# CILAB-MA/gpudrive_lab

Measured on AMD Instinct MI355X. Metric: agent-steps/sec at 1024 worlds x 64 agents; achieved HBM GB/s on obs kernel, higher is better.
Workload: dtype f32

## Files before the change

gpudrive_lab_amd/csrc/engine.cpp:

```cpp
#include <hip/hip_runtime.h>

#include <algorithm>
#include <cmath>
#include <cstdlib>
#include <cstdio>
#include <cstring>
#include <map>
#include <memory>
#include <stdexcept>
#include <atomic>
#include <exception>
#include <string>
#include <thread>
#include <vector>

#include "dev_mem.hpp"
#include "engine.hpp"
#include "gd_math.hpp"
#include "scene.hpp"
#ifdef GD_CLOCKS
namespace gd { void set_clocks_read(unsigned long long *out); void step_clocks_read(unsigned long long *out); }
#endif
#ifndef GD_GRID_MIN_CELL
#define GD_GRID_MIN_CELL 16.f
// ... 127 lines not shown
    std::vector<int32_t> deleted;
    std::vector<WorldHost> world_host;
    int cu_count = 256;
    Growable<float2, 320, 640> road_xy;
    Growable<Float8, 320, 640> road_aux, road_rec;
    Growable<gd::RoadBox, 0, 64> boxes;
    Growable<int32_t, 0, 64> cell_off, cell_items;
    Growable<float4, 0, 64> cell_hdr;
    Growable<int32_t, 0, 64> rcell_off;
    Growable<uint16_t, 64, 128> rcell_items, rcell_pos;
    Growable<float2, 64, 128> rcell_xy;
    Growable<float4, 0, 64> road_blk;
    int32_t *d_road_off = nullptr, *d_box_off = nullptr, *d_blk_off = nullptr;
    gd::GridHdr *d_grid = nullptr, *d_rgrid = nullptr;
    float4 *d_road_bbox = nullptr;
    float *d_road_rbmax = nullptr;
    static constexpr int kRing = 8;
    PinnedFlags h_flags[kRing];
    Event flag_ev[kRing];
    int ring_pos = 0;
    static constexpr size_t kEvRing = 32;
    Stream side;
    Event ev_fork, ev_join;
    size_t lin_cap = 0;
    int32_t *d_row_of_slot = nullptr, *d_slot_of_row = nullptr, *d_row_count = nullptr;
    int32_t *d_lin_list = nullptr, *d_lin_list_dyn = nullptr;
    bool full_pass_next = false;
    int64_t lin_static_agents = 0;
    int64_t host_skipped = 0;
    bool rk_possible = false;
    bool rk_alloc = false;

    bool ensure_rank_buffers() {
        if (rk_alloc) return true;
        const size_t WA = static_cast<size_t>(W) * A;
        std::vector<gd::DevMem> mine;
        gd::DevSim n = d;
        try {
            alloc_into(mine, n.rk_E, WA * GD_RANK_CAP + 64);
            alloc_into(mine, n.rk_spc, WA * GD_RANK_SPL);
            if (std::getenv("GPUDRIVE_RANK_ALLOC_FAIL") != nullptr)
                throw HipError("GPUDRIVE_RANK_ALLOC_FAIL: simulated allocation failure of the rank replay's buffers");
            alloc_into(mine, n.rk_kt, WA * GD_RANK_KT);
            alloc_into(mine, n.rk_heap, WA * GD_RANK_HEAP_DW);
            alloc_into(mine, n.rk_cpe, WA * GD_RANK_NCP);
            alloc_into(mine, n.rk_n, WA);
            alloc_into(mine, n.rk_fallback, WA / 32);
            alloc_into(mine, n.rk_streak, WA / 32);
            alloc_into(mine, n.cp_road, 2 * WA * GD_RANK_NCP);
            alloc_into(mine, n.cp_T, 2 * WA * GD_RANK_NCP);
            alloc_into(mine, n.cp_hdr, 2 * WA);
            alloc_into(mine, n.rk_cp, WA * GD_RANK_NCP);
            alloc_into(mine, n.rk_tl, WA);
            alloc_into(mine, n.rk_hist, 544);
            alloc_into(mine, n.rk_ticket, WA);
            alloc_into(mine, n.rk_order, WA);
            alloc_into(mine, n.rk_list, 8 * WA);
            n.rk_nlong = static_cast<int>(std::max<size_t>(WA / 4, 64));
            alloc_into(mine, n.rk_longlist, n.rk_nlong);
            alloc_into(mine, n.rk_longslot, WA);
            alloc_into(mine, n.rk_E_long, static_cast<size_t>(n.rk_nlong) * GD_RANK_CAP_LONG + 64);
            alloc_into(mine, n.rk_kt_long, static_cast<size_t>(n.rk_nlong) * GD_RANK_KT_LONG);
            internal.reserve(internal.size() + mine.size());
        } catch (const HipError &) {
            (void)hipGetLastError();
            rk_possible = false;
            d.rk_on = 0;
            return false;
        }
        for (gd::DevMem &m : mine) internal.push_back(std::move(m));
        d = n;
        rk_alloc = true;
        return true;
    }
    bool timing = false;
    std::vector<EventPair> ev_pool[gd::KERNEL_TIMED];
    size_t ev_head[gd::KERNEL_TIMED] = {};
    size_t ev_used[gd::KERNEL_TIMED] = {};
    double ev_ms[gd::KERNEL_TIMED] = {};
    int64_t ev_launches[gd::KERNEL_TIMED] = {};

    ~gd_sim() {
        (void)hipDeviceSynchronize();
        if (step_graph) (void)hipGraphExecDestroy(step_graph);
    }

    template <typename T>
    static void alloc_into(std::vector<gd::DevMem> &into, T *&field, size_t count) {
        const size_t bytes = std::max<size_t>(count * sizeof(T), 16);
        into.emplace_back(bytes);
        HIP_CHECK(hipMemset(into.back().get(), 0, bytes));
        field = static_cast<T *>(into.back().get());
    }
    template <typename T>
    T *alloc_internal(size_t count) {
        T *p = nullptr;
        alloc_into(internal, p, count);
        return p;
    }

    void collect_timing(int k, size_t keep = 0) {
        while (ev_used[k] > keep) {
            const EventPair &e = ev_pool[k][ev_head[k]];
            float ms = 0.f;
            if (hipEventSynchronize(e.stop.get()) == hipSuccess && hipEventElapsedTime(&ms, e.start.get(), e.stop.get()) == hipSuccess) {
                ev_ms[k] += ms;
                ev_launches[k]++;
// ... 523 lines not shown
            for (int c = 0; c < nc; c++) off[c + 1] += off[c];
            std::vector<int32_t> fill(off.begin(), off.end() - 1);
            for (size_t r = 0; r < n; r++) items[fill[cell_of[r]]++] = static_cast<uint16_t>(r);
        }
        world.rgrid = g;
        world.rcell_off = std::move(off);
        world.rcell_items = std::move(items);
    }

    void upload_road_grids() {
        size_t ncell = 0, nitem = 0;
        std::vector<gd::GridHdr> hdr(W);
        for (int w = 0; w < W; w++) {
            world_host[w].rgrid.cell_base = static_cast<int>(ncell);
            world_host[w].rgrid.item_base = static_cast<int>(nitem);
            hdr[w] = world_host[w].rgrid;
            ncell += world_host[w].rcell_off.size();
            nitem += world_host[w].rcell_items.size();
        }
        rcell_off.fit(ncell, d.rcell_off);
        rcell_items.fit(nitem, d.rcell_items);
        rcell_xy.fit(nitem, d.rcell_xy);
        rcell_pos.fit(nitem, d.rcell_pos);
        std::vector<int32_t> co(ncell);
        std::vector<uint16_t> ci(nitem);
        std::vector<float> cxy(nitem * 2);
        std::vector<uint16_t> cpos(nitem);
        for (int w = 0; w < W; w++) {
            const WorldHost &x = world_host[w];
            std::copy(x.rcell_off.begin(), x.rcell_off.end(), co.begin() + hdr[w].cell_base);
            std::copy(x.rcell_items.begin(), x.rcell_items.end(), ci.begin() + hdr[w].item_base);
            for (size_t k = 0; k < x.rcell_items.size(); k++) {
                const size_t r = x.rcell_items[k], o = (static_cast<size_t>(hdr[w].item_base) + k) * 2;
                cxy[o] = x.xy[2 * r];
                cxy[o + 1] = x.xy[2 * r + 1];
                cpos[static_cast<size_t>(hdr[w].item_base) + r] = static_cast<uint16_t>(k);
            }
        }
        rcell_off.upload(co.data(), ncell);
        rcell_items.upload(ci.data(), nitem);
        rcell_xy.upload(cxy.data(), nitem);
        rcell_pos.upload(cpos.data(), nitem);
        HIP_CHECK(hipMemcpy(d_rgrid, hdr.data(), sizeof(gd::GridHdr) * W, hipMemcpyHostToDevice));
        std::vector<float> prev(static_cast<size_t>(W) * A * 4, 0.f);
        for (size_t i = 0; i < static_cast<size_t>(W) * A; i++) prev[i * 4 + 2] = INFINITY;
        HIP_CHECK(hipMemcpy(d.knn_prev, prev.data(), prev.size() * sizeof(float), hipMemcpyHostToDevice));
    }

    void reset_rank_state() {
        HIP_CHECK(hipMemset(d.cp_hdr, 0, sizeof(float4) * 2 * static_cast<size_t>(W) * A));
        HIP_CHECK(hipMemset(d.rk_fallback, 0, sizeof(int32_t) * (static_cast<size_t>(W) * A / 32)));
        HIP_CHECK(hipMemset(d.rk_streak, 0, sizeof(int32_t) * (static_cast<size_t>(W) * A / 32)));
        HIP_CHECK(hipMemset(d.rk_hist, 0, sizeof(int32_t) * GD_RANK_AUDIT));
    }

    void do_reset(const std::vector<int32_t> &flags) {
        upload_flags(d.reset_flags, flags);
        reset_flagged(false);
    }

    void reset_flagged(bool gated) {
        d.gate_any = gated ? 1 : 0;
        if (!gated) full_pass_next = false;
        try {
            launch(gd::KERNEL_RESET, false);
            run_rest(false);
        } catch (...) {
            d.gate_any = 0;
            throw;
        }
        d.gate_any = 0;
    }
};

namespace {

template <typename F>
int guarded(F &&f) {
    try {
        f();
        return GD_OK;
    } catch (const HipError &e) {
        return fail(GD_ERR_DEVICE, e.what());
    } catch (const std::invalid_argument &e) {
        const std::string m = e.what();
        return fail(m.find("cannot open") != std::string::npos ? GD_ERR_IO : GD_ERR_INVALID, m);
    } catch (const std::exception &e) {
        return fail(GD_ERR_PARSE, e.what());
    }
}

}

extern "C" {

const char *gd_version(void) { return "gpudrive_amd 0.1 (gfx950)"; }
const char *gd_last_error(void) { return g_last_error.c_str(); }

void gd_default_params(gd_params *p) {
    std::memset(p, 0, sizeof(*p));
    p->collisionBehaviour = GD_COLLISION_AGENT_STOP;
    p->maxNumControlledAgents = 10000;
    p->IgnoreNonVehicles = 0;
    p->roadObservationAlgorithm = GD_ROADS_K_NEAREST;
    p->initOnlyValidAgentsAtFirstStep = 1;
    p->isStaticAgentControlled = 0;
// ... 105 lines not shown
        d.resp = s->alloc_internal<int32_t>(WA);
        d.sel_idx = s->alloc_internal<uint16_t>(static_cast<size_t>(WA) * GD_MAP_OBS_K);
        d.sel_hdr = s->alloc_internal<float4>(static_cast<size_t>(WA) * 2);
        d.sel_slot = s->alloc_internal<uint8_t>(static_cast<size_t>(WA) * GD_MAP_OBS_K);
        d.reset_flags = s->alloc_internal<int32_t>(W);
        d.rebuilt_flags = s->alloc_internal<int32_t>(W);
        d.any_reset = s->alloc_internal<int32_t>(1);
        d.gate_any = 0;
        d.road_off = s->d_road_off = s->alloc_internal<int32_t>(W + 1);
        d.live_list = s->alloc_internal<int32_t>(WA);
        d.live_count = 0;
        d.set_groups = s->alloc_internal<int32_t>(WA);
        d.set_group_count = 0;
        d.wave_order = s->alloc_internal<int32_t>(static_cast<size_t>(W) * (A / GD_MAP_OBS_AW));
        d.wave_cost = s->alloc_internal<uint32_t>(static_cast<size_t>(W) * (A / GD_MAP_OBS_AW));
        d.box_off = s->d_box_off = s->alloc_internal<int32_t>(W + 1);
        d.grid = s->d_grid = s->alloc_internal<gd::GridHdr>(W);
        d.rgrid = s->d_rgrid = s->alloc_internal<gd::GridHdr>(W);
        d.knn_prev = s->alloc_internal<float4>(WA);
        d.road_bbox = s->d_road_bbox = s->alloc_internal<float4>(W);
        d.road_rbmax = s->d_road_rbmax = s->alloc_internal<float>(W);
        d.bev_dirty = s->alloc_internal<int32_t>(WA);
        d.bev_list = s->alloc_internal<int32_t>(WA);
        d.bev_count = s->alloc_internal<int32_t>(2);
        d.bev_all_dirty = 0;
        HIP_CHECK(hipMemset(d.bev_dirty, 1, sizeof(int32_t) * WA));
        d.lidar_dirty = s->alloc_internal<int32_t>(WA);
        d.lidar_head = s->alloc_internal<float>(WA);
        HIP_CHECK(hipMemset(d.lidar_dirty, 1, sizeof(int32_t) * WA));
        HIP_CHECK(hipMemset(d.lidar_head, 0xff, sizeof(float) * WA));
        d.lin_apw = 2;
        if (const char *e = std::getenv("GPUDRIVE_LIN_AGENTS_PER_WAVE")) d.lin_apw = std::min(A / 4, std::max(1, std::atoi(e)));
        s->lin_cap = (static_cast<size_t>(W) + 64) * static_cast<size_t>(A) + 8 * 4 * static_cast<size_t>(d.lin_apw) + 64;
        s->d_lin_list = s->alloc_internal<int32_t>(s->lin_cap);
        s->d_lin_list_dyn = s->alloc_internal<int32_t>(s->lin_cap);
        d.lin_list = s->d_lin_list; d.lin_list_dyn = s->d_lin_list_dyn;
        d.lin_blocks = 0; d.lin_blocks_dyn = 0; d.lin_dyn_off = 0;
        d.lin_on = std::getenv("GPUDRIVE_LINEAR_LEGACY") == nullptr ? 1 : 0;
        d.pose_stamp = s->alloc_internal<uint4>(WA);
        d.pose_skip = std::getenv("GPUDRIVE_NO_POSE_SKIP") == nullptr ? 1 : 0;
        d.stat_skipped = s->alloc_internal<unsigned long long>(GD_SKIP_SLOTS);
        s->d_row_of_slot = s->alloc_internal<int32_t>(WA);
        s->d_slot_of_row = s->alloc_internal<int32_t>(WA);
        s->d_row_count = s->alloc_internal<int32_t>(1);
        d.bad_actions = s->alloc_internal<unsigned long long>(1);
        d.blk_off = s->d_blk_off = s->alloc_internal<int32_t>(W + 1);
        d.warm_k = 0;
        d.warm_all = 0;
        d.warm_flags = s->alloc_internal<int32_t>(W);
        d.warm_count = s->alloc_internal<unsigned long long>(1);
        d.rk_on = 0;
        d.rk_dbg = 0;
        d.rk_min_roads = 1536;
        s->rk_possible = GD_MAP_OBS_AW == 32 && cfg->knn_order != GD_KNN_SET_ORDER &&
                         params->roadObservationAlgorithm == GD_ROADS_K_NEAREST && std::getenv("GPUDRIVE_NO_RANK_REPLAY") == nullptr;
#ifdef GD_DIAG
        if (const char *e = std::getenv("GPUDRIVE_RANK_DBG")) d.rk_dbg = std::atoi(e);
#endif
        for (int i = 0; i < gd_sim::kRing; i++) {
            void *pinned = nullptr;
            HIP_CHECK(hipHostMalloc(&pinned, sizeof(int32_t) * W, hipHostMallocDefault));
            s->h_flags[i].reset(static_cast<int32_t *>(pinned));
            s->flag_ev[i] = make_event(hipEventDisableTiming);
        }
        std::vector<int> all(W);
        for (int w = 0; w < W; w++) all[w] = w;
        s->rebuild_worlds(all);
        s->do_reset(std::vector<int32_t>(W, 1));
        HIP_CHECK(hipStreamSynchronize(s->stream));
    });
    if (rc != GD_OK) return rc;
    *out = s.release();
    return GD_OK;
}

void gd_destroy(gd_sim *sim) { delete sim; }

int gd_step(gd_sim *s) {
    if (!s) return fail(GD_ERR_INVALID, "gd_step: null sim");
    return guarded([&]() { s->step(); });
}

int gd_reset(gd_sim *s, const int32_t *idx, int32_t n) {
    if (!s || (n > 0 && !idx)) return fail(GD_ERR_INVALID, "gd_reset: bad argument");
    std::vector<int32_t> flags(s->W, 0);
    for (int i = 0; i < n; i++) {
        if (idx[i] < 0 || idx[i] >= s->W) return fail(GD_ERR_INVALID, "gd_reset: world index out of range");
        flags[idx[i]] = 1;
    }
    return guarded([&]() { s->do_reset(flags); });
}

int gd_set_maps(gd_sim *s, const char *const *scenes, int32_t n) {
    if (!s || !scenes) return fail(GD_ERR_INVALID, "gd_set_maps: null argument");
    if (n != s->W) return fail(GD_ERR_INVALID, "gd_set_maps: len(maps) must equal the number of worlds");
    const std::vector<std::string> old_scenes = s->scenes;
    const std::vector<int32_t> old_deleted = s->deleted;
    const int rc = guarded([&]() {
        for (int w = 0; w < n; w++) {
            if (!scenes[w]) throw std::invalid_argument("gd_set_maps: null scene path");
            s->scenes[w] = scenes[w];
        }
        std::fill(s->deleted.begin(), s->deleted.end(), -1);
        std::vector<int> all(s->W);
        for (int w = 0; w < s->W; w++) all[w] = w;
        s->rebuild_worlds(all);
// ... 1070 lines not shown
    if (!s) return fail(GD_ERR_INVALID, "gd_set_stream: null sim");
    return guarded([&]() {
        HIP_CHECK(hipStreamSynchronize(s->stream));
        s->drop_graph();
        HIP_CHECK(hipStreamSynchronize(s->side.get()));
        s->stream = static_cast<hipStream_t>(stream);
        s->d.split_partner = (s->stream != nullptr && std::getenv("GPUDRIVE_SPLIT_PARTNER") != nullptr) ? 1 : 0;
    });
}

int gd_attach_bev(gd_sim *s, float *bev) {
    if (!s || !bev) return fail(GD_ERR_INVALID, "gd_attach_bev: null argument");
    return guarded([&]() {
        if (s->d.bev && s->d.bev != bev) throw std::runtime_error("gd_attach_bev: a BEV tensor is already attached");
        HIP_CHECK(hipStreamSynchronize(s->stream));
        s->drop_graph();
        s->exported[GD_T_BEV] = bev;
        s->d.bev = bev;
        HIP_CHECK(hipMemsetAsync(s->d.bev_dirty, 1, sizeof(int32_t) * static_cast<size_t>(s->W) * s->A, s->stream));
        if (!s->params.disableClassicalObs) s->launch(gd::KERNEL_BEV, false);
    });
}

int gd_stat(gd_sim *s, int32_t which, int64_t *out) {
#ifdef GD_CLOCKS
    if (s && out && which >= 22 && which <= 29) {
        static unsigned long long clk[8];
        if (which == 22) gd::set_clocks_read(clk);
        *out = (int64_t)clk[which - 22];
        return GD_OK;
    }
#endif
#ifdef GD_CLOCKS
    if (s && out && which >= 32 && which <= 43) {
        static unsigned long long clk[12];
        if (which == 32) gd::step_clocks_read(clk);
        *out = (int64_t)clk[which - 32];
        return GD_OK;
    }
#endif
#ifdef GD_CLOCKS
    if (s && out && which >= 1000 && which < 1256) {
        *out = 0;
        if (s->rk_alloc) {
            int32_t v = 0;
            (void)hipStreamSynchronize(s->stream);
            if (hipMemcpy(&v, s->d.rk_hist + 256 + (which - 1000), sizeof(v), hipMemcpyDeviceToHost) != hipSuccess)
                return fail(GD_ERR_DEVICE, "gd_stat: reading the replay clocks failed");
            *out = v;
        }
        return GD_OK;
    }
#endif
#if defined(GD_DIAG) || defined(GD_CLOCKS)
    constexpr int32_t kLastStat = 20;
#else
    constexpr int32_t kLastStat = 7;
#endif
    if (s && out && which == 30) {
        std::vector<unsigned long long> v(GD_SKIP_SLOTS, 0);
        (void)hipStreamSynchronize(s->stream);
        if (hipMemcpy(v.data(), s->d.stat_skipped, sizeof(unsigned long long) * v.size(), hipMemcpyDeviceToHost) != hipSuccess ||
            hipMemset(s->d.stat_skipped, 0, sizeof(unsigned long long) * v.size()) != hipSuccess)
            return fail(GD_ERR_DEVICE, "gd_stat: reading the skip counters failed");
        unsigned long long sum = 0;
        for (unsigned long long x : v) sum += x;
        *out = static_cast<int64_t>(sum) + s->host_skipped;
        s->host_skipped = 0;
        return GD_OK;
    }
    if (s && out && which == 31) {
        int32_t c = 0;
        (void)hipStreamSynchronize(s->stream);
        if (hipMemcpy(&c, s->d.bev_count, sizeof(c), hipMemcpyDeviceToHost) != hipSuccess)
            return fail(GD_ERR_DEVICE, "gd_stat: reading the raster count failed");
        *out = c;
        return GD_OK;
    }
    if (s && out && which == 44) {
        std::vector<int32_t> f(static_cast<size_t>(s->W) * s->A), n(static_cast<size_t>(s->W) * 2);
        (void)hipStreamSynchronize(s->stream);
        if (hipMemcpy(f.data(), s->d.lidar_dirty, sizeof(int32_t) * f.size(), hipMemcpyDeviceToHost) != hipSuccess ||
            hipMemcpy(n.data(), s->d.shape, sizeof(int32_t) * n.size(), hipMemcpyDeviceToHost) != hipSuccess)
            return fail(GD_ERR_DEVICE, "gd_stat: reading the LiDAR flags failed");
        int64_t c = 0;
        for (int w = 0; w < s->W; w++)
            for (int a = 0; a < n[static_cast<size_t>(w) * 2] && a < s->A; a++) c += f[static_cast<size_t>(w) * s->A + a] != 0;
        *out = c;
        return GD_OK;
    }
    if (s && out && which == 45) {
        unsigned long long v = 0;
        (void)hipStreamSynchronize(s->stream);
        if (hipMemcpy(&v, s->d.bad_actions, sizeof(v), hipMemcpyDeviceToHost) != hipSuccess)
            return fail(GD_ERR_DEVICE, "gd_stat: reading the action counter failed");
        *out = static_cast<int64_t>(v);
        return GD_OK;
    }
    if (s && out && which == 46) {
        unsigned long long v = 0;
        (void)hipStreamSynchronize(s->stream);
        if (hipMemcpy(&v, s->d.warm_count, sizeof(v), hipMemcpyDeviceToHost) != hipSuccess)
            return fail(GD_ERR_DEVICE, "gd_stat: reading the warm-up counter failed");
        *out = static_cast<int64_t>(v);
        return GD_OK;
    }
// ... 180 lines not shown
```

gpudrive_lab_amd/csrc/engine.hpp:

```cpp
#pragma once
#include <hip/hip_runtime.h>

#include <cstdint>

#include "../../include/gpudrive_amd.h"

#ifndef GD_MAP_OBS_AW
#define GD_MAP_OBS_AW 32
#endif

#define GD_RANK_CAP 1280
#define GD_RANK_NCP 40
#define GD_RANK_HEAP_DW 104
#define GD_RANK_CAP_LONG 2560
#define GD_RANK_KT_LONG 164
#define GD_RH_LONG 537
#define GD_RANK_NCH 320
#define GD_RANK_SPL 256
#define GD_RANK_KT 84
#define GD_RANK_AUDIT 536
#define GD_LIN_BLK 16
#define GD_SKIP_SLOTS 4096

#ifdef GD_DIAG
#define GD_DIAG_IS(field, value) ((field) == (value))
#else
#define GD_DIAG_IS(field, value) false
#endif

namespace gd {

enum { KERNEL_STATE = 0, KERNEL_MAP_OBS = 1, KERNEL_LIDAR = 2, KERNEL_BEV = 3, KERNEL_PARTNER = 4, KERNEL_RESET = 5, KERNEL_PADDING = 6, KERNEL_TIMED = 5 };

struct GridHdr {
    float ox, oy, inv_cell;
    int nx, ny;
    int cell_base;
    int item_base;
    int pad;
};

struct DevSim {
    int W, A;
    int knn_order;
    int set_fused_rows;
    int32_t *live_list;
    int live_count;
    int32_t *set_groups;
    int set_group_count;
    int set_apw;
    float lidar_half_angle;
    float radius_key_max;
    gd_params p;
    float *action, *reward, *self_obs, *abs_obs, *partner, *agent_map, *map_obs, *lidar, *bev, *traj, *means;
    int32_t *done, *info, *shape, *controlled, *resp_export, *metadata, *deleted, *map_name, *scenario_id;
    uint32_t *steps;
    float *px, *py, *pz, *qw, *qz, *vx, *vy, *vz;
    int32_t *collided;
    float *len, *wid, *hgt, *sc0, *sc1, *goal_x, *goal_y;
    int32_t *etype, *agent_id, *resp;
    uint16_t *sel_idx;
    float4 *sel_hdr;
    uint8_t *sel_slot;
    int32_t *reset_flags, *rebuilt_flags;
    int32_t *any_reset;
    int gate_any;
    const int32_t *road_off;
    int32_t *wave_order;
    uint32_t *wave_cost;
// ... 1 lines not shown
    const float4 *road_aux;
    const float4 *road_rec;
    const int32_t *box_off;
    const float4 *boxes;
    const GridHdr *grid;
    const int32_t *cell_off;
    const int32_t *cell_items;
    const float4 *cell_hdr;
    const GridHdr *rgrid;
    const int32_t *rcell_off;
    const uint16_t *rcell_items;
    const float2 *rcell_xy;
    const uint16_t *rcell_pos;
    float4 *knn_prev;
    const int32_t *lin_list, *lin_list_dyn;
    int lin_blocks, lin_blocks_dyn;
    int lin_dyn_off;
    const float4 *road_blk;
    const int32_t *blk_off;
    int lin_apw;
    int lin_on;
    uint4 *pose_stamp;
    int pose_skip;
    int32_t *bev_dirty;
    int32_t *bev_list;
    int32_t *bev_count;
    int bev_all_dirty;
    int32_t *lidar_dirty;
    float *lidar_head;
    float *pack;
    int pack_only;
    const int32_t *row_of_slot, *slot_of_row;
    int n_rows;
    int pack_rows;
    unsigned long long *bad_actions;
    unsigned long long *stat_skipped;
    int split_partner;
    int step_dbg;
    int rk_on;
    int rk_max_roads;
    int rk_min_roads;
    int rk_dbg;
    uint16_t *rk_E;
    int rk_nlong;
    int32_t *rk_longlist;
    int32_t *rk_longslot;
    uint16_t *rk_E_long;
    float *rk_kt_long;
    uint16_t *rk_spc;
    float *rk_kt;
    uint32_t *rk_heap;
    uint16_t *rk_cpe;
    int32_t *rk_hist;
    int32_t *rk_ticket;
    int32_t *rk_order;
    int32_t *rk_list;
    uint2 *rk_cp;
    float *rk_tl;
    const float4 *road_bbox;
    const float *road_rbmax;
    int32_t *rk_n;
    int32_t *rk_fallback;
    int32_t *rk_streak;
    uint16_t *cp_road;
    float *cp_T;
    float4 *cp_hdr;
    int warm_k;
    int warm_all;
    int32_t *warm_flags;
    unsigned long long *warm_count;
    const float *pack_weights;
};

void launch_kernel(const DevSim &d, hipStream_t st, int which, bool move);
void launch_map_obs(const DevSim &d, hipStream_t st, bool move);
void launch_map_obs_rank(const DevSim &d, hipStream_t st);
void launch_map_obs_linear(const DevSim &d, hipStream_t st, bool move);
void launch_bev(const DevSim &d, hipStream_t st);
void launch_lidar(const DevSim &d, hipStream_t st);
void launch_pack_obs(const DevSim &d, hipStream_t st, float *out);
void launch_expert_actions(const DevSim &d, hipStream_t st, float *actions, float *pos, float *vel, float *yaw, int *valid);
void launch_set_log_actions(const DevSim &d, hipStream_t st, int t);
void launch_episode_step(const DevSim &d, hipStream_t st, const gd_episode_config &c, const gd_episode_buffers &b);
void launch_draw_weights(const DevSim &d, hipStream_t st, const gd_episode_config &c, const gd_episode_buffers &b,
                         const int32_t *worlds, int n);
void launch_pack_obs_rows(const DevSim &d, hipStream_t st, float *out,
                          const float *weights);
void launch_learner_rows(hipStream_t st, const uint8_t *mask, size_t slots, int32_t *row_of_slot, int32_t *slot_of_row,
                         int32_t *count);
void launch_discrete_actions(const DevSim &d, hipStream_t st, const int64_t *indices, const float *table, int n_actions);
void launch_pack_obs_conditioned(const DevSim &d, hipStream_t st, const float *weights, float *out);
void launch_record(const DevSim &d, hipStream_t st, const gd_record_buffers &b, int t, bool pre);
void launch_bc_rollout_row(const DevSim &d, hipStream_t st, const gd_bc_rollout_buffers &b, int t, int num_stack);
void launch_bc_rollout_actions(const DevSim &d, hipStream_t st, const gd_bc_rollout_buffers &b, int t);
void launch_bc_rollout_post(const DevSim &d, hipStream_t st, const gd_bc_rollout_buffers &b, int t, bool more);
void launch_bc_rollout_summary(hipStream_t st, const gd_bc_rollout_buffers &b);
void launch_policy_rollout_actions(const DevSim &d, hipStream_t st, const gd_policy_rollout_buffers &b, int t);
void launch_policy_rollout_book(const DevSim &d, hipStream_t st, const gd_policy_rollout_buffers &b, int t);
void launch_policy_rollout_finish(const DevSim &d, hipStream_t st, const gd_policy_rollout_buffers &b, int n_steps);
void launch_il_index(const gd_il_dataset &ds, hipStream_t st, int64_t rows, int32_t *counts, int32_t *kept,
                     const int64_t *entry_offset, const int64_t *kept_ordinal, int32_t *entries);
void launch_il_batch(const gd_il_dataset &ds, hipStream_t st, const gd_il_batch_buffers &b,
                     int split);
void launch_il_future(const gd_il_dataset &ds, const gd_il_future &fu, hipStream_t st, const gd_il_future_buffers &b,
                      int split);
void launch_rollout_store(const gd_rollout &ro, hipStream_t st, const float *obs, const float *value, const int64_t *action,
// ... 57 lines not shown
```

gpudrive_lab_amd/csrc/map_obs_rank.hip:

```cpp
#include <hip/hip_runtime.h>

#include <algorithm>
#include <type_traits>

#include "engine.hpp"
#include "gd_math.hpp"
#include "rank_cand.hpp"
#include "rank_heap.hpp"

namespace gd {

namespace {

constexpr int K = GD_MAP_OBS_K;
constexpr int CAP = GD_RANK_CAP;
constexpr int NCP = GD_RANK_NCP;
constexpr int SPL = GD_RANK_SPL;
constexpr int KT = GD_RANK_KT;
constexpr int TILE = 32;
constexpr int CAP_LONG = GD_RANK_CAP_LONG;
template <int CAP_T>
struct RankGeo {
    static constexpr bool LONG = CAP_T > CAP;
    static constexpr int NG = CAP_T / 64;
// ... 301 lines not shown
static_assert(sizeof(RankLds<CAP>) <= 10240 && sizeof(RankLds<CAP_LONG>) <= 20480, "sixteen / eight waves per CU");
constexpr int LSTN = (GD_MAX_ROAD_ENTITIES + GD_LIN_BLK - 1) / GD_LIN_BLK + 15;
constexpr int LSTN4 = (LSTN + 3) & ~3;
static_assert(LSTN4 <= 1024 && NCP < 64 && rank_cand::CHUNK % GD_LIN_BLK == 0 && 64 % GD_LIN_BLK == 0, "block and count share 16 bits; a block inside one chunk; whole blocks per pass");
constexpr size_t CAND_TABLES = LSTN4 * sizeof(unsigned short) + (NCP + 1) * sizeof(float);
static_assert(CAND_TABLES <= sizeof(RankLds<CAP>::cnt2) && CAND_TABLES <= sizeof(RankLds<CAP_LONG>::cnt2), "the tables fit the idle counters of both instantiations");
constexpr int CP_EPL = ((GD_MAX_ROAD_ENTITIES + rank_cand::CHUNK - 1) / rank_cand::CHUNK + 63) / 64;
static_assert(64 * CP_EPL * (sizeof(unsigned int) + sizeof(uint2)) <= sizeof(float) * CAP, "the chunk table fits the candidate keys of both instantiations");

struct RankIn {
    int i, state, r0, R, b0, li;
    float ex, ey, iw, iz, t_last;
    unsigned int cfirst;
    float cthr;
};
template <typename T>
__device__ __forceinline__ T uniform_load(const T *p) {
    return *reinterpret_cast<const __attribute__((address_space(4))) T *>(reinterpret_cast<uintptr_t>(p));
}
template <int A_T>
__device__ __forceinline__ RankIn rank_fetch(const DevSim &d, const int *list, int li, int count, int lane) {
    RankIn in;
    in.li = li;
    in.i = li < count ? uniform_load(list + li) : 0;
    in.state = li < count ? uniform_load(d.rk_n + in.i) : 0;
    const int w = in.i / A_T;
    in.r0 = uniform_load(d.road_off + w);
    in.R = uniform_load(d.road_off + w + 1) - in.r0;
    in.ex = uniform_load(d.px + in.i); in.ey = uniform_load(d.py + in.i);
    in.iw = uniform_load(d.qw + in.i); in.iz = -uniform_load(d.qz + in.i);
    in.t_last = uniform_load(d.rk_tl + in.i);
    in.b0 = uniform_load(d.blk_off + w);
    uint2 cp = make_uint2(rank_cand::NO_CP, __float_as_uint(__builtin_inff()));
    if (in.state == 1 && lane < NCP) cp = stream_load(d.rk_cp + (size_t)in.i * NCP + (unsigned int)lane);
    in.cfirst = cp.x;
    in.cthr = __uint_as_float(cp.y);
    return in;
}

#ifdef GD_CLOCKS
struct PhaseClock {
    unsigned int prev, sum[8];
    __device__ __forceinline__ void mark(int n) {
        const unsigned int t = (unsigned int)__builtin_amdgcn_s_memtime();
        sum[n] += t - prev;
        prev = t;
    }
};
#define GD_PHASE(n) clk.mark(n)
#else
struct PhaseClock {};
#define GD_PHASE(n)
#endif
template <int A_T, int CAP_T>
__device__ __forceinline__ void rank_agent(const DevSim &d, const RankIn &in, int lane, RankLds<CAP_T> &L, PhaseClock &clk, int next_entry,
                                           int count, const int *list, RankIn &nxt) {
    using G = RankGeo<CAP_T>;
    constexpr int NB = G::NB, NLIN = G::NLIN, NMAX = G::NMAX;
    constexpr unsigned int TM = (1u << G::RSH) - 1u;
    if (__builtin_amdgcn_readfirstlane(in.state) != 1) {
        nxt = rank_fetch<A_T>(d, list, next_entry, count, lane);
        return;
    }
    auto uni = [](int v) -> int { return __builtin_amdgcn_readfirstlane(v); };
    auto unif = [](float v) -> float { return __int_as_float(__builtin_amdgcn_readfirstlane(__float_as_int(v))); };
    const int i = uni(in.i), r0 = uni(in.r0), R = uni(in.R);
    const int group = i / 32;
    constexpr int NG = G::NG;

    const float ex = unif(in.ex), ey = unif(in.ey), iw = unif(in.iw), iz = unif(in.iz);
    unsigned short *const lst = reinterpret_cast<unsigned short *>(L.cnt2);
    float *const tthr = reinterpret_cast<float *>(L.cnt2) + LSTN4 / 2;
    const unsigned int cfirst = in.cfirst;
    if (lane < NCP) tthr[lane + 1] = in.cthr;
    if (lane == 63) tthr[0] = __builtin_inff();
    const float creach = rank_cand::block_reach(in.cthr);
    const int nblk = (R + GD_LIN_BLK - 1) / GD_LIN_BLK;
    const int nch = rank_cand::chunks_of(R), epl = (nch + 63) >> 6;
    unsigned int *const tmax = reinterpret_cast<unsigned int *>(L.c.ckey);
    uint2 *const tcp = reinterpret_cast<uint2 *>(L.c.ckey + 64 * CP_EPL);
#pragma unroll
    for (int u = 0; u < CP_EPL; u++)
        if (u < epl) tmax[u * 64 + lane] = 0u;
    wave_sync();
    if (lane < NCP && rank_cand::cp_table_takes(cfirst, nch)) atomicMax(&tmax[rank_cand::cp_table_chunk(cfirst)], rank_cand::cp_table_entry(lane));
    wave_sync();
    {
        int own[CP_EPL], run = 0;
#pragma unroll
        for (int u = 0; u < CP_EPL; u++) own[u] = u < epl ? (int)tmax[lane * epl + u] : 0;
#pragma unroll
        for (int u = 0; u < CP_EPL; u++) { run = max(run, own[u]); own[u] = run; }
        const int before = __builtin_amdgcn_ds_bpermute(((lane - 1) & 63) << 2, wave_incl_max_nonneg(run));
#pragma unroll
        for (int u = 0; u < CP_EPL; u++)
            if (u < epl) {
                const int cnt = lane ? max(own[u], before) : own[u];
                const int reach = __builtin_amdgcn_ds_bpermute(((cnt - 1) & 63) << 2, __float_as_int(creach));
                tcp[lane * epl + u] = make_uint2((unsigned int)cnt, (unsigned int)reach);
            }
    }
    wave_sync();
    const float4 *blk = d.road_blk + uni(in.b0);
    int nsv = 0;
    constexpr int CU = 4;
#pragma clang loop unroll(disable)
    for (int b0 = 0; b0 < nblk; b0 += 64 * CU) {
        float4 c[CU];
        uint2 cp[CU];
#pragma unroll
        for (int u = 0; u < CU; u++) {
            const int bc = min(b0 + u * 64 + lane, nblk - 1);
            c[u] = blk[(unsigned int)bc];
            cp[u] = tcp[rank_cand::chunk_base_of_block(bc, GD_LIN_BLK) / rank_cand::CHUNK];
        }
        static_assert(CU == 4, "operand list");
        asm volatile("" : "+v"(c[0].x), "+v"(c[0].y), "+v"(c[0].z), "+v"(c[1].x), "+v"(c[1].y), "+v"(c[1].z), "+v"(c[2].x), "+v"(c[2].y), "+v"(c[2].z),
                     "+v"(c[3].x), "+v"(c[3].y), "+v"(c[3].z));
#pragma unroll
        for (int u = 0; u < CU; u++) {
            const int bb = b0 + u * 64;
            if (bb < nblk) {
                const int b = bb + lane;
                const bool sv = b < nblk && rank_cand::block_survives(b, GD_LIN_BLK, K, c[u].x, c[u].y, c[u].z, ex, ey, __uint_as_float(cp[u].y));
                const unsigned long long m = wave_ballot(sv);
                const int upto = nsv + __popcll(m);
                if (upto <= LSTN4) {
                    if (sv) lst[nsv + bits_below_lane(m)] = (unsigned short)((unsigned int)b | cp[u].x << 10);
                    nsv = upto;
                } else if (lane == 0) {
                    atomicAdd(&d.rk_hist[GD_RANK_AUDIT], 1);
                }
            }
        }
    }
    wave_sync();
    int nin = 0;
    {
        constexpr int BPP = 64 / GD_LIN_BLK, PB = 2;
        const int np = (nsv + BPP - 1) / BPP, nfast = np - 1;
        const int sub = lane / GD_LIN_BLK, o = lane % GD_LIN_BLK;
        const float2 *rxy = d.road_xy + r0;
        auto store = [&](bool cand, int r, float key, unsigned long long m, bool guard) {
            const int pos = nin + bits_below_lane(m);
            if (cand && (!guard || pos < CAP_T)) {
                L.c.cidx[pos] = (unsigned short)r;
                L.c.ckey[pos] = key;
            }
            nin += __popcll(m);
        };
        int p = 0;
        if (nfast >= 2 * PB) {
            const unsigned int *lsub = reinterpret_cast<const unsigned int *>(L.cnt2) + sub / 2;
            const unsigned int sh = (unsigned int)(sub & 1) * 16u;
            const unsigned int o8 = (unsigned int)o * (unsigned int)sizeof(float2);
            static_assert(BPP == 4, "two words per pass");
            struct Ents { unsigned int e[PB]; };
            struct Batch { unsigned int off[PB]; float thr[PB]; float2 xy[PB]; };
            auto entries = [&](Ents &en, int p0) {
#pragma unroll
                for (int u = 0; u < PB; u++) en.e[u] = lsub[min(p0 + u, nfast - 1) * (BPP / 2)];
            };
            auto issue = [&](Batch &bt, const Ents &en) {
#pragma unroll
                for (int u = 0; u < PB; u++) {
                    bt.off[u] = __builtin_amdgcn_ubfe(en.e[u], sh, 10u) * (unsigned int)(GD_LIN_BLK * sizeof(float2)) + o8;
                    bt.thr[u] = tthr[__builtin_amdgcn_ubfe(en.e[u], sh + 10u, 6u)];
                    bt.xy[u] = *reinterpret_cast<const float2 *>(reinterpret_cast<const char *>(rxy) + bt.off[u]);
                }
            };
            auto take = [&](const Batch &bt) {
#pragma unroll
                for (int u = 0; u < PB; u++) {
                    const int r = (int)(bt.off[u] / (unsigned int)sizeof(float2));
                    __builtin_assume(r >= 0 && r < R);
                    const bool cand = rank_cand::is_candidate(r, K, R, bt.xy[u].x, bt.xy[u].y, ex, ey, bt.thr[u]);
                    store(cand, r, ego_dist2(ex, ey, iw, iz, bt.xy[u].x, bt.xy[u].y), wave_ballot(cand), false);
                }
            };
            Ents ea, eb;
            Batch ba, bb;
            entries(ea, 0);
            entries(eb, PB);
            issue(ba, ea);
#pragma clang loop unroll(disable)
            for (; p + 2 * PB <= nfast && nin + 2 * PB * 64 <= CAP_T; p += 2 * PB) {
                issue(bb, eb);
                entries(ea, p + 2 * PB);
                take(ba);
// ... 252 lines not shown
                const int first = b ? (int)cur16[b - 1] : 0, end = (int)cur16[b];
                float kg = 0.f;
                for (int m = first; m < end; m++) kg = (int)L.s.spos[m] == p ? L.s.skey[m] : kg;
                for (int m = first; m < end; m++) tie += (L.s.skey[m] == kg ? 1 : 0) & ((int)L.s.spos[m] < p ? 1 : 0);
            }
            too_many_ties |= tie > (int)TM ? 1 : 0;
#pragma unroll
            for (int k = 0; k < NG; k++) ci[k] |= k == g ? (tie & (int)TM) << 16 : 0;
        }
    }
    wave_sync();
    GD_PHASE(5);
    if (GD_DIAG_IS(d.rk_dbg, 5)) return;
    if (__ballot(too_many_ties != 0) != 0ull) {
        if (lane == 0) {
            d.rk_n[i] = 0;
            d.rk_ticket[i] = ticket | RK_TIES;
            d.rk_fallback[group] = 1;
        }
        return;
    }
    unsigned short *const E_row = G::LONG ? d.rk_E_long + (size_t)uni(in.li) * CAP_LONG : d.rk_E + (size_t)i * CAP;
    const unsigned int ulane = (unsigned int)lane;
#pragma unroll
    for (int g = 0; g < NG; g++) {
        if (g * 64 < nin) {
            if (g * 64 + lane < nin) {
                const unsigned int e = (unsigned int)ci[g] >> 16;
                stream_store((unsigned short)e, E_row + (g * 64u + ulane));
                const int slot = (int)(e >> G::RSH) - 1 + (int)(e & TM);
                if (slot < SPL) L.spc[slot] = (unsigned short)(ci[g] & 0xffff);
            }
        }
    }
    wave_sync();
    {
        static_assert(SPL == 256, "four slots per lane");
        const uint2 v = reinterpret_cast<const uint2 *>(L.spc)[lane];
        stream_store(v, reinterpret_cast<uint2 *>(d.rk_spc + (size_t)i * SPL) + ulane);
    }
    if (lane == 0) {
        d.rk_n[i] = nin | (nle << 16) | (has_tie ? 1 << 28 : 0) | (G::LONG ? 1 << 29 : 0);
        if (G::LONG) d.rk_longslot[i] = uni(in.li);
        d.rk_ticket[i] = ticket;
    }
    GD_PHASE(6);
}

template <int A_T, int CAP_T>
__global__ __launch_bounds__(64, CAP_T > CAP ? 2 : 4) void k_knn_rank(DevSim d) {
    if (d.gate_any && *d.any_reset == 0) return;
    __shared__ RankLds<CAP_T> L;
    constexpr bool LONG = RankGeo<CAP_T>::LONG;
    const int stride = LONG ? (int)gridDim.x : (int)(gridDim.x >> 3);
    const int xcd = blockIdx.x & 7;
    const int count = LONG ? min(uniform_load(d.rk_hist + GD_RH_LONG), d.rk_nlong) : uniform_load(d.rk_hist + 528 + xcd);
    const int *list = LONG ? d.rk_longlist : d.rk_list + (size_t)xcd * d.W * A_T;
    int t = LONG ? (int)blockIdx.x : (int)(blockIdx.x >> 3);
    RankIn cur = rank_fetch<A_T>(d, list, t, count, threadIdx.x);
    PhaseClock clk;
#ifdef GD_CLOCKS
    for (int k = 0; k < 8; k++) clk.sum[k] = 0u;
    clk.prev = (unsigned int)__builtin_amdgcn_s_memtime();
#endif
    for (; t < count; t += stride) {
        RankIn nxt;
        GD_PHASE(0);
        int lane_v = threadIdx.x;
        asm volatile("" : "+v"(lane_v));
        rank_agent<A_T, CAP_T>(d, cur, lane_v, L, clk, t + stride, count, list, nxt);
        wave_sync();
        cur = nxt;
    }
#ifdef GD_CLOCKS
    if (threadIdx.x == 0)
        for (int k = 0; k < 8; k++) atomicAdd(reinterpret_cast<unsigned int *>(&d.rk_hist[516 + k]), clk.sum[k] >> 8);
#endif
}

#ifndef GD_RANK_AWR
#define GD_RANK_AWR 64
#endif
constexpr int AWR = GD_RANK_AWR;
typedef unsigned int __attribute__((may_alias)) heap_u32;
typedef unsigned short __attribute__((may_alias)) heap_u16;
struct RankHeap {
    heap_u32 *pr;
    __device__ __forceinline__ unsigned int pair(int j) const { return pr[j * AWR]; }
    __device__ __forceinline__ unsigned int get(int g) const {
        return reinterpret_cast<const heap_u16 *>(pr + (g >> 1) * AWR)[g & 1];
    }
    __device__ __forceinline__ void set(int g, unsigned int v) const {
        reinterpret_cast<heap_u16 *>(pr + (g >> 1) * AWR)[g & 1] = (unsigned short)v;
    }
    __device__ __forceinline__ void set_pair(int j, unsigned int v) const { pr[j * AWR] = v; }
};
static_assert(rank_heap::NPAIR == 128, "s_pair of k_knn_replay");

__global__ __launch_bounds__(256) void k_knn_order(DevSim d) {
    if (d.gate_any && *d.any_reset == 0) return;
    __shared__ int s_part[4];
    __shared__ int s_start[256];
    const int tl = threadIdx.x;
    const int c = d.rk_hist[tl];
    const int incl = wave_incl_scan(c);
    if ((tl & 63) == 63) s_part[tl >> 6] = incl;
    __syncthreads();
    int before = 0;
    for (int k = 0; k < (tl >> 6); k++) before += s_part[k];
    s_start[tl] = before + incl - c;
    if (blockIdx.x == 0 && tl == 255) {
        d.rk_hist[512] = before + incl;
        d.rk_hist[513]++;
        for (int x = 0; x < 8; x++) d.rk_hist[528 + x] = 0;
        d.rk_hist[GD_RH_LONG] = 0;
    }
#ifdef GD_CLOCKS
    if (blockIdx.x == 0) d.rk_hist[256 + tl] = 0;
#endif
    __syncthreads();
    const int t = blockIdx.x * 256 + tl;
    if (t >= d.live_count) return;
    const int i = d.live_list[t];
    const int ticket = d.rk_ticket[i];
    if (ticket < 0) return;
    d.rk_order[audited(d, s_start[(ticket >> 20) & 255] + (ticket & 0xfffff), d.W * d.A)] = i;
}

#ifdef GD_CLOCKS
struct ReplayClock {
    unsigned int prev, first, ph[5];
    __device__ __forceinline__ void start() { first = prev = (unsigned int)__builtin_amdgcn_s_memrealtime(); }
    __device__ __forceinline__ void mark(int n) {
        const unsigned int t = (unsigned int)__builtin_amdgcn_s_memrealtime();
        ph[n] = t - prev;
        prev = t;
    }
};
#define GD_RPHASE(n) rclk.mark(n)
#else
#define GD_RPHASE(n)
#endif
__global__ __launch_bounds__(64) void k_knn_replay(DevSim d) {
    if (d.gate_any && *d.any_reset == 0) return;
    const int lane = threadIdx.x;
#ifdef GD_CLOCKS
    ReplayClock rclk;
    rclk.start();
#endif
    if (blockIdx.x == 0)
        for (int k = 0; k < 4; k++) d.rk_hist[k * 64 + lane] = 0;
    const int li = blockIdx.x * AWR + lane;
    constexpr int NPAIR = 128;
    __shared__ unsigned int s_pair[NPAIR * AWR];
    const RankHeap H{reinterpret_cast<heap_u32 *>(s_pair) + (lane % AWR)};
    int i = 0, n = 0, has_tie = 0, is_long = 0;
    if (lane < AWR && li < d.rk_hist[512]) {
        i = d.rk_order[li];
        const int packed = d.rk_n[i];
        n = packed & 0xffff;
        has_tie = (packed >> 28) & 1;
        is_long = (packed >> 29) & 1;
        if (d.rk_fallback[i / 32] != 0) n = 0;
    }
    const bool on = n >= K;
    if (__ballot(on) == 0ull) return;
    const unsigned short *E = (on && is_long) ? d.rk_E_long + (size_t)d.rk_longslot[i] * CAP_LONG : d.rk_E + (size_t)i * CAP;
    const unsigned int tm = is_long ? 15u : 31u;
// ... 252 lines not shown
#pragma unroll
        for (int k = 0; k < WL; k++) { own[k] = bm[lane * WL + k]; sum += __popc(own[k]); }
        int run = wave_incl_scan(sum) - sum;
#pragma unroll
        for (int k = 0; k < WL; k++) { s_wp[wave][lane * WL + k] = (unsigned short)run; run += __popc(own[k]); }
    }
    wave_sync();
#pragma unroll
    for (int ps = 0; ps < NP; ps++) {
        const int t = ps * 64 + lane;
        if (t < m) {
            const int rd = min(max(road[ps], 0), R - 1);
            const int place = (int)s_wp[wave][rd >> 5] + __popc(bm[rd >> 5] & ((1u << (rd & 31)) - 1u));
            s_sorted[wave][audited(d, place, m)] = (unsigned int)rd | (unsigned int)t << 16;
        }
    }
    wave_sync();
#pragma unroll
    for (int ps = 0; ps < NP; ps++) {
        const int q = ps * 64 + lane;
        if (q < K) {
            const unsigned int v = q < m ? s_sorted[wave][q] : (unsigned int)q << 16;
            d.sel_idx[(size_t)i * K + q] = (unsigned short)(v & 0xffffu);
            d.sel_slot[(size_t)i * K + q] = (unsigned char)(v >> 16);
        }
    }
    const bool at_start = steps_left == (uint32_t)GD_EPISODE_LEN;
    const size_t WA = (size_t)d.W * A_T;
    if (lane < ncp) {
        (void)audited(d, cp_slot, n);
        d.cp_T[(size_t)i * NCP + lane] = cp_t;
        if (at_start) {
            d.cp_T[(WA + i) * NCP + lane] = cp_t;
            d.cp_road[(WA + i) * NCP + lane] = cp_r;
        }
    }
    if (lane == 0) {
        d.rk_streak[i / 32] = 0;
        d.cp_hdr[i] = make_float4(ex, ey, __int_as_float(ncp), 0.f);
        if (at_start) d.cp_hdr[WA + i] = make_float4(ex, ey, __int_as_float(ncp), 0.f);
        d.sel_hdr[(size_t)i * 2] = make_float4(ex, ey, qw, qz);
        d.sel_hdr[(size_t)i * 2 + 1] = make_float4(__int_as_float(m), __int_as_float(r0), __int_as_float(1), 0.f);
    }
}

}

#ifndef GD_RANK_LONG_GRID
#define GD_RANK_LONG_GRID 2048
#endif
void launch_map_obs_rank(const DevSim &d, hipStream_t st) {
    if (d.live_count == 0) return;
    const dim3 glong(std::min(std::max(d.rk_nlong, 1), GD_RANK_LONG_GRID));
    const dim3 gr(std::min((d.live_count + 7) / 8 * 8, 256 * 8 * 4)), g4((d.live_count + 3) / 4), gw(d.W * (d.A / 64));
    if (d.A == 64) {
        hipLaunchKernelGGL((k_knn_scan<64>), gw, dim3(256), 0, st, d);
        hipLaunchKernelGGL((k_knn_rank<64, CAP>), gr, dim3(64), 0, st, d);
        if (d.rk_nlong > 0) hipLaunchKernelGGL((k_knn_rank<64, CAP_LONG>), glong, dim3(64), 0, st, d);
    } else {
        hipLaunchKernelGGL((k_knn_scan<128>), gw, dim3(256), 0, st, d);
        hipLaunchKernelGGL((k_knn_rank<128, CAP>), gr, dim3(64), 0, st, d);
        if (d.rk_nlong > 0) hipLaunchKernelGGL((k_knn_rank<128, CAP_LONG>), glong, dim3(64), 0, st, d);
    }
    hipLaunchKernelGGL(k_knn_order, dim3((d.live_count + 255) / 256), dim3(256), 0, st, d);
    hipLaunchKernelGGL(k_knn_replay, dim3((d.live_count + AWR - 1) / AWR), dim3(64), 0, st, d);
    if (d.A == 64) hipLaunchKernelGGL((k_knn_finish<64>), g4, dim3(256), 0, st, d);
    else hipLaunchKernelGGL((k_knn_finish<128>), g4, dim3(256), 0, st, d);
}

}
```

Measured before the change: 67.38 million.

## Replace static strided agent assignment in rank kernel with atomic work-stealing cursor

The ranking kernel now draws its next agent index from a per-XCD atomic cursor instead of striding by a fixed grid share, when there are more agents than waves. This balances uneven per-agent ranking work across waves, so waves no longer wait on a few slow strided chains. The cost is one atomic per agent and a prefetch index that depends on the atomic result. Also adds an env knob for grid size and optional per-wave clock instrumentation.

```diff
diff --git a/gpudrive_lab_amd/csrc/engine.cpp b/gpudrive_lab_amd/csrc/engine.cpp
--- a/gpudrive_lab_amd/csrc/engine.cpp
+++ b/gpudrive_lab_amd/csrc/engine.cpp
@@ -203,7 +203,7 @@
             alloc_into(mine, n.cp_hdr, 2 * WA);
             alloc_into(mine, n.rk_cp, WA * GD_RANK_NCP);
             alloc_into(mine, n.rk_tl, WA);
-            alloc_into(mine, n.rk_hist, 544);
+            alloc_into(mine, n.rk_hist, GD_RH_ALLOC);
             alloc_into(mine, n.rk_ticket, WA);
             alloc_into(mine, n.rk_order, WA);
             alloc_into(mine, n.rk_list, 8 * WA);
@@ -833,6 +833,7 @@
         HIP_CHECK(hipMemset(d.rk_fallback, 0, sizeof(int32_t) * (static_cast<size_t>(W) * A / 32)));
         HIP_CHECK(hipMemset(d.rk_streak, 0, sizeof(int32_t) * (static_cast<size_t>(W) * A / 32)));
         HIP_CHECK(hipMemset(d.rk_hist, 0, sizeof(int32_t) * GD_RANK_AUDIT));
+        HIP_CHECK(hipMemset(d.rk_hist + GD_RH_LONG, 0, sizeof(int32_t) * (GD_RH_SIZE - GD_RH_LONG)));
     }
 
     void do_reset(const std::vector<int32_t> &flags) {
@@ -1044,6 +1045,8 @@
         d.rk_on = 0;
         d.rk_dbg = 0;
         d.rk_min_roads = 1536;
+        d.rk_waves = 0;
+        if (const char *e = std::getenv("GPUDRIVE_RANK_WAVES")) d.rk_waves = std::min(std::max((std::atoi(e) + 7) / 8 * 8, 8), GD_RANK_GRID);
         s->rk_possible = GD_MAP_OBS_AW == 32 && cfg->knn_order != GD_KNN_SET_ORDER &&
                          params->roadObservationAlgorithm == GD_ROADS_K_NEAREST && std::getenv("GPUDRIVE_NO_RANK_REPLAY") == nullptr;
 #ifdef GD_DIAG
@@ -2220,6 +2223,19 @@
         return GD_OK;
     }
 #endif
+#ifdef GD_WAVE_CLOCKS
+    if (s && out && which >= 2000 && which < 2000 + 3 * GD_RANK_GRID) {
+        *out = 0;
+        if (s->rk_alloc) {
+            int32_t v = 0;
+            (void)hipStreamSynchronize(s->stream);
+            if (hipMemcpy(&v, s->d.rk_hist + GD_RH_WAVES + (which - 2000), sizeof(v), hipMemcpyDeviceToHost) != hipSuccess)
+                return fail(GD_ERR_DEVICE, "gd_stat: reading the ranking waves' clocks failed");
+            *out = v;
+        }
+        return GD_OK;
+    }
+#endif
 #if defined(GD_DIAG) || defined(GD_CLOCKS)
     constexpr int32_t kLastStat = 20;
 #else
diff --git a/gpudrive_lab_amd/csrc/engine.hpp b/gpudrive_lab_amd/csrc/engine.hpp
--- a/gpudrive_lab_amd/csrc/engine.hpp
+++ b/gpudrive_lab_amd/csrc/engine.hpp
@@ -15,6 +15,19 @@
 #define GD_RANK_CAP_LONG 2560
 #define GD_RANK_KT_LONG 164
 #define GD_RH_LONG 537
+#define GD_RH_CURSOR 544
+#define GD_RH_CURSOR_STRIDE 32
+#define GD_RH_SIZE (GD_RH_CURSOR + 8 * GD_RH_CURSOR_STRIDE)
+#define GD_RANK_GRID (256 * 8 * 4)
+#ifdef GD_CLOCKS
+#define GD_WAVE_CLOCKS
+#endif
+#ifdef GD_WAVE_CLOCKS
+#define GD_RH_WAVES GD_RH_SIZE
+#define GD_RH_ALLOC (GD_RH_WAVES + 3 * GD_RANK_GRID)
+#else
+#define GD_RH_ALLOC GD_RH_SIZE
+#endif
 #define GD_RANK_NCH 320
 #define GD_RANK_SPL 256
 #define GD_RANK_KT 84
@@ -122,6 +135,7 @@
     uint32_t *rk_heap;
     uint16_t *rk_cpe;
     int32_t *rk_hist;
+    int rk_waves;
     int32_t *rk_ticket;
     int32_t *rk_order;
     int32_t *rk_list;
diff --git a/gpudrive_lab_amd/csrc/map_obs_rank.hip b/gpudrive_lab_amd/csrc/map_obs_rank.hip
--- a/gpudrive_lab_amd/csrc/map_obs_rank.hip
+++ b/gpudrive_lab_amd/csrc/map_obs_rank.hip
@@ -377,14 +377,19 @@
 struct PhaseClock {};
 #define GD_PHASE(n)
 #endif
+__device__ __forceinline__ int rank_draw(int *cursor, int lane) {
+    int e = 0;
+    if (lane == 0) e = atomicAdd(cursor, 1);
+    return e;
+}
 template <int A_T, int CAP_T>
-__device__ __forceinline__ void rank_agent(const DevSim &d, const RankIn &in, int lane, RankLds<CAP_T> &L, PhaseClock &clk, int next_entry,
+__device__ __forceinline__ void rank_agent(const DevSim &d, const RankIn &in, int lane, RankLds<CAP_T> &L, PhaseClock &clk, int drawn,
                                            int count, const int *list, RankIn &nxt) {
     using G = RankGeo<CAP_T>;
     constexpr int NB = G::NB, NLIN = G::NLIN, NMAX = G::NMAX;
     constexpr unsigned int TM = (1u << G::RSH) - 1u;
     if (__builtin_amdgcn_readfirstlane(in.state) != 1) {
-        nxt = rank_fetch<A_T>(d, list, next_entry, count, lane);
+        nxt = rank_fetch<A_T>(d, list, __builtin_amdgcn_readfirstlane(drawn), count, lane);
         return;
     }
     auto uni = [](int v) -> int { return __builtin_amdgcn_readfirstlane(v); };
@@ -460,6 +465,7 @@
         }
     }
     wave_sync();
+    const int next_entry = uni(drawn);
     int nin = 0;
     {
         constexpr int BPP = 64 / GD_LIN_BLK, PB = 2;
@@ -818,29 +824,51 @@
     if (d.gate_any && *d.any_reset == 0) return;
     __shared__ RankLds<CAP_T> L;
     constexpr bool LONG = RankGeo<CAP_T>::LONG;
-    const int stride = LONG ? (int)gridDim.x : (int)(gridDim.x >> 3);
     const int xcd = blockIdx.x & 7;
     const int count = LONG ? min(uniform_load(d.rk_hist + GD_RH_LONG), d.rk_nlong) : uniform_load(d.rk_hist + 528 + xcd);
     const int *list = LONG ? d.rk_longlist : d.rk_list + (size_t)xcd * d.W * A_T;
-    int t = LONG ? (int)blockIdx.x : (int)(blockIdx.x >> 3);
+    int *const cursor = d.rk_hist + GD_RH_CURSOR + xcd * GD_RH_CURSOR_STRIDE;
+    const int share = LONG ? (int)gridDim.x : (int)(gridDim.x >> 3), mine = LONG ? (int)blockIdx.x : (int)(blockIdx.x >> 3);
+    const bool fixed = LONG || count <= share;
+#ifdef GD_WAVE_CLOCKS
+    int turns = 0;
+    if (!LONG && threadIdx.x == 0) {
+        d.rk_hist[GD_RH_WAVES + blockIdx.x] = (int)__builtin_amdgcn_s_memrealtime();
+        d.rk_hist[GD_RH_WAVES + 2 * GD_RANK_GRID + blockIdx.x] = 0;
+    }
+#endif
+    if (fixed && mine >= count) return;
+    int t = fixed ? mine : __builtin_amdgcn_readfirstlane(rank_draw(cursor, threadIdx.x));
     RankIn cur = rank_fetch<A_T>(d, list, t, count, threadIdx.x);
     PhaseClock clk;
 #ifdef GD_CLOCKS
     for (int k = 0; k < 8; k++) clk.sum[k] = 0u;
     clk.prev = (unsigned int)__builtin_amdgcn_s_memtime();
 #endif
-    for (; t < count; t += stride) {
+    while (t < count) {
         RankIn nxt;
         GD_PHASE(0);
         int lane_v = threadIdx.x;
         asm volatile("" : "+v"(lane_v));
-        rank_agent<A_T, CAP_T>(d, cur, lane_v, L, clk, t + stride, count, list, nxt);
+        const int drawn = fixed ? t + share : rank_draw(cursor, lane_v);
+        rank_agent<A_T, CAP_T>(d, cur, lane_v, L, clk, drawn, count, list, nxt);
         wave_sync();
         cur = nxt;
+        t = __builtin_amdgcn_readfirstlane(nxt.li);
+#ifdef GD_WAVE_CLOCKS
+        turns++;
+#endif
     }
 #ifdef GD_CLOCKS
     if (threadIdx.x == 0)
         for (int k = 0; k < 8; k++) atomicAdd(reinterpret_cast<unsigned int *>(&d.rk_hist[516 + k]), clk.sum[k] >> 8);
+#endif
+#ifdef GD_WAVE_CLOCKS
+    if (!LONG && threadIdx.x == 0) {
+        asm volatile("s_waitcnt vmcnt(0)" ::: "memory");
+        d.rk_hist[GD_RH_WAVES + GD_RANK_GRID + blockIdx.x] = (int)__builtin_amdgcn_s_memrealtime();
+        d.rk_hist[GD_RH_WAVES + 2 * GD_RANK_GRID + blockIdx.x] = turns;
+    }
 #endif
 }
 
@@ -880,6 +908,7 @@
         d.rk_hist[513]++;
         for (int x = 0; x < 8; x++) d.rk_hist[528 + x] = 0;
         d.rk_hist[GD_RH_LONG] = 0;
+        for (int x = 0; x < 8; x++) d.rk_hist[GD_RH_CURSOR + x * GD_RH_CURSOR_STRIDE] = 0;
     }
 #ifdef GD_CLOCKS
     if (blockIdx.x == 0) d.rk_hist[256 + tl] = 0;
@@ -1238,7 +1267,7 @@
 void launch_map_obs_rank(const DevSim &d, hipStream_t st) {
     if (d.live_count == 0) return;
     const dim3 glong(std::min(std::max(d.rk_nlong, 1), GD_RANK_LONG_GRID));
-    const dim3 gr(std::min((d.live_count + 7) / 8 * 8, 256 * 8 * 4)), g4((d.live_count + 3) / 4), gw(d.W * (d.A / 64));
+    const dim3 gr(d.rk_waves > 0 ? d.rk_waves : std::min((d.live_count + 7) / 8 * 8, GD_RANK_GRID)), g4((d.live_count + 3) / 4), gw(d.W * (d.A / 64));
     if (d.A == 64) {
         hipLaunchKernelGGL((k_knn_scan<64>), gw, dim3(256), 0, st, d);
         hipLaunchKernelGGL((k_knn_rank<64, CAP>), gr, dim3(64), 0, st, d);
```

After: 69.51 million, median of 6. +3.2%, better.
